# Adamtaranto/frisk

Hardware: AMD Instinct MI355X
Metric: windows/sec (k=1..8, w=5kb, s=1kb) (higher is better)
Workload: dtype u8/u4 counts + f64 scores

## Files before the change

### frisk_amd/csrc/frisk_abi.hip

```cpp
#include <hip/hip_runtime.h>
#include <zlib.h>
#include <dlfcn.h>

#include <algorithm>
#include <cmath>
#include <cstdio>
#include <cstdlib>
#include <cstring>
#include <new>
#include <string>
#include <atomic>
#include <chrono>
#include <thread>
#include <vector>

#include "frisk_hip.h"
#include "frisk_device.h"
#include "profile_kernels.h"
#include "scan_launch.h"
#include "scan_schedule.h"
#include "ring_rows.h"
#include "synth_kernel.h"
#include "table_text.h"
#include "fasta_index.h"
// ... 10 lines not shown
    hipError_t reserve(size_t n) {
        if (n <= cap) return hipSuccess;
        if (p) { hipError_t e = hipFree(p); p = nullptr; cap = 0; if (e != hipSuccess) return e; }
        size_t want = n + n / 8 + 64;
        hipError_t e = hipMalloc(reinterpret_cast<void**>(&p), want * sizeof(T));
        if (e != hipSuccess) { p = nullptr; return e; }
        cap = want;
        return hipSuccess;
    }
    void release() { if (p) (void)hipFree(p); p = nullptr; cap = 0; }
};

}

struct frisk_ctx {
    int device = 0;
    int kmin = 1, kmax = 8;
    int64_t nprof = 0;
    int num_cu = 256;
    hipStream_t stream = nullptr;
    hipEvent_t ev0 = nullptr, ev1 = nullptr;
    double ms[3] = {-1.0, -1.0, -1.0};
    std::string err;

    struct Batch {
        int32_t n_seq = 0;
        std::vector<int64_t> seq_off, seq_len;
        std::vector<std::string> seq_name;
        int64_t padded_len = 0;
        bool have_seq = false;
        DevBuf<uint8_t> d_ascii;
        DevBuf<uint32_t> d_codes, d_inv, d_low;
        struct Tile {
            int32_t scaf;
            int64_t size;
            int64_t base0;
            int64_t j0, ncand;
            int32_t kind;
            int64_t own0, own1;
        };
        int width_hint = 0, hint_w = 0, hint_inc = 0, hint_side = 0;
        bool tiled = false;
        std::vector<Tile> tiles;
        int32_t tile_w = 0, tile_inc = 0;
        uint32_t tile_flags = 0;
        int64_t cand_begin = 0, cand_end = 0;
        std::vector<std::string> g_name;
        std::vector<int64_t> g_len;
        std::vector<int64_t> piece_end;
        std::vector<hipEvent_t> piece_ev;
        bool streaming = false;
        DevBuf<int64_t> d_runs;
        std::vector<uint32_t, frisk_fasta::NoInitAlloc<uint32_t>> h_codes;
        frisk_pack2::Runs h_runs;
        bool have_host2 = false;
        int64_t* h_pads = nullptr;
        size_t h_pads_cap = 0;
        void release() {
            d_ascii.release(); d_codes.release(); d_inv.release(); d_low.release(); d_runs.release();
            if (h_pads) (void)hipHostFree(h_pads);
            h_pads = nullptr; h_pads_cap = 0;
            for (hipEvent_t e : piece_ev) (void)hipEventDestroy(e);
            piece_ev.clear();
        }
    };
    Batch bat[2];
    int cur = 0;
    Batch& b() { return bat[cur]; }
    const Batch& b() const { return bat[cur]; }
    hipStream_t copy_stream = nullptr;
    static constexpr int PIN_N = 8;
    static constexpr size_t PIN_BYTES = size_t(16) << 20;
    void* pin_buf[PIN_N] = {nullptr, nullptr, nullptr, nullptr, nullptr, nullptr, nullptr, nullptr};
    hipEvent_t pin_ev[PIN_N] = {nullptr, nullptr, nullptr, nullptr, nullptr, nullptr, nullptr, nullptr};
    bool pin_busy[PIN_N] = {false, false, false, false, false, false, false, false};
    hipStream_t tail_stream = nullptr;
    hipEvent_t ev_fork = nullptr, ev_tail_kernels = nullptr, ev_tail_done = nullptr;
    hipEvent_t staged_ev = nullptr;
    hipEvent_t slot_free_ev = nullptr;
    bool slot_ev_set = false;
    bool staged = false;

    DevBuf<int64_t> d_raw, d_cnt, d_sym;
    DevBuf<double> d_ig, d_logtab, d_logtab64, d_logtab32, d_rctab;
    DevBuf<int64_t> d_ovf_list, d_ovf_list2;
    uint64_t ig_gen = 1, ring_gen = 0;
    DevBuf<double> d_ig_ring;
    DevBuf<unsigned int> d_verdict;
    DevBuf<unsigned int> d_ovf_count;
    int64_t scan_stat[5] = {0, 0, 0, 0, 0};
    DevBuf<uint32_t> d_big;
    DevBuf<int64_t> d_meta;
    int64_t* h_meta = nullptr;
    bool profile_final = false;
    bool ms_pending[3] = {false, false, false};
    hipEvent_t evp0 = nullptr, evp1 = nullptr;

    DevBuf<ScafDesc> d_desc;
    std::vector<ScafDesc> h_desc;
    int32_t plan_w = -1, plan_inc = -1;
    uint32_t plan_flags = 0;
    int64_t plan_ncand = 0;
    int64_t plan_maxwin = 0;
    DevBuf<int32_t> o_seq;
    DevBuf<int64_t> o_start, o_stop, o_meta;
    DevBuf<uint32_t> o_status, o_counts;
    DevBuf<double> o_kld, o_gc, o_pi, o_si, o_cri, o_sw, o_sg, o_ivom;
    DevBuf<double> o_block;
    void* h_block = nullptr;
    size_t h_block_cap = 0;
    double* want_ivom = nullptr;
};

namespace {

int fail(frisk_ctx* c, int code, const std::string& msg) {
    if (c) c->err = msg;
    return code;
}

#define HIPC(ctx, call)                                                                         \
    do {                                                                                        \
        hipError_t e_ = (call);                                                                 \
        if (e_ != hipSuccess)                                                                   \
            return fail((ctx), FRISK_E_HIP, std::string(#call) + ": " + hipGetErrorString(e_)); \
    } while (0)

int64_t profile_len(int kmin, int kmax) { return table_offset(kmin, kmax + 1); }

int grid_for(int64_t items, int per_block, int max_blocks) {
    int64_t b = (items + per_block - 1) / per_block;
    if (b < 1) b = 1;
    if (b > max_blocks) b = max_blocks;
    return int(b);
}

int settle_stream(frisk_ctx* c);

int layout_batch(frisk_ctx* c, frisk_ctx::Batch& B, const int64_t* lens, int32_t n_seq) {
    if (n_seq < 0) return fail(c, FRISK_E_ARG, "n_seq < 0");
    for (int32_t s = 0; s < n_seq; ++s)
        if (lens[s] < 0) return fail(c, FRISK_E_ARG, "negative scaffold length");
    if (&B == &c->b()) {
        const int rc = settle_stream(c);
        if (rc) return rc;
    }
    B.seq_off.assign(size_t(n_seq), 0);
    B.seq_len.assign(lens, lens + n_seq);
    B.seq_name.assign(size_t(n_seq), std::string());
    int64_t pos = 0;
    for (int32_t s = 0; s < n_seq; ++s) {
        B.seq_off[size_t(s)] = pos;
        pos += lens[s] + 1;
    }
    B.padded_len = (pos + 31) / 32 * 32;
    if (B.padded_len == 0) B.padded_len = 32;
    B.n_seq = n_seq;
    B.have_seq = false;
    B.width_hint = 0;
    B.tiled = false;
    B.tiles.clear(); B.g_name.clear(); B.g_len.clear();
    B.streaming = false;
    if (B.have_host2) {
        B.have_host2 = false;
        decltype(B.h_codes)().swap(B.h_codes);
        B.h_runs = frisk_pack2::Runs();
// ... 177 lines not shown

}

extern "C" {

const char* frisk_version(void) { return "frisk_hip 0.1 (gfx950)"; }

int frisk_supported(int kmin, int kmax, int64_t max_window) {
    return (kmin >= 1 && kmin <= kmax && kmax <= FRISK_MAX_K && max_window >= 1 && max_window <= 0x7FFFFFFF) ? 1 : 0;
}

int frisk_create(int device, int kmin, int kmax, frisk_ctx** out) {
    if (!out) return FRISK_E_ARG;
    *out = nullptr;
    frisk_ctx* c = new (std::nothrow) frisk_ctx();
    if (!c) return FRISK_E_HIP;
    *out = c;
    if (kmin < 1 || kmin > kmax || kmax > FRISK_MAX_K)
        return fail(c, FRISK_E_ARG, "word sizes must satisfy 1 <= kmin <= kmax <= 12");
    c->device = device;
    c->kmin = kmin;
    c->kmax = kmax;
    c->nprof = profile_len(kmin, kmax);
    int ndev = 0;
    HIPC(c, hipGetDeviceCount(&ndev));
    if (device < 0 || device >= ndev) return fail(c, FRISK_E_HIP, "no such HIP device");
    HIPC(c, hipSetDevice(device));
    hipDeviceProp_t prop;
    HIPC(c, hipGetDeviceProperties(&prop, device));
    if (std::string(prop.gcnArchName).rfind("gfx950", 0) != 0)
        return fail(c, FRISK_E_HIP, std::string("libfrisk_hip is built for gfx950 only; device is ") + prop.gcnArchName);
    c->num_cu = prop.multiProcessorCount;
    HIPC(c, hipStreamCreateWithFlags(&c->stream, hipStreamNonBlocking));
    HIPC(c, hipStreamCreateWithFlags(&c->copy_stream, hipStreamNonBlocking));
    HIPC(c, hipEventCreateWithFlags(&c->staged_ev, hipEventDisableTiming));
    HIPC(c, hipEventCreateWithFlags(&c->slot_free_ev, hipEventDisableTiming));
    HIPC(c, hipStreamCreateWithFlags(&c->tail_stream, hipStreamNonBlocking));
    HIPC(c, hipEventCreateWithFlags(&c->ev_fork, hipEventDisableTiming));
    HIPC(c, hipEventCreateWithFlags(&c->ev_tail_kernels, hipEventDisableTiming));
    HIPC(c, hipEventCreateWithFlags(&c->ev_tail_done, hipEventDisableTiming));
    HIPC(c, hipEventCreate(&c->ev0));
    HIPC(c, hipEventCreate(&c->ev1));
    HIPC(c, c->d_raw.reserve(size_t(c->nprof) + 4));
    HIPC(c, c->d_cnt.reserve(size_t(c->nprof) + 4));
    HIPC(c, c->d_sym.reserve(size_t(c->nprof)));
    HIPC(c, c->d_ig.reserve(size_t(1) << (2 * kmax)));
    HIPC(c, c->d_meta.reserve(4));
    HIPC(c, hipHostMalloc(reinterpret_cast<void**>(&c->h_meta), 4 * sizeof(int64_t), hipHostMallocDefault));
    HIPC(c, hipEventCreate(&c->evp0));
    HIPC(c, hipEventCreate(&c->evp1));
    HIPC(c, hipMemsetAsync(c->d_raw.p, 0, (size_t(c->nprof) + 4) * sizeof(int64_t), c->stream));
    {
        double tab[2 * FRISK_LOGTAB_N];
        for (int nbin : {FRISK_LOGTAB_N, 64, 32}) {
            for (int i = 0; i < nbin; ++i) {
                const double ci = 0.5 + (double(i) + 0.5) / (2.0 * nbin);
                const double u = 1.0 / ci;
                tab[2 * i] = u;
                tab[2 * i + 1] = double(-logl((long double)u));
            }
            DevBuf<double>& dst = nbin == 64 ? c->d_logtab64 : (nbin == 32 ? c->d_logtab32 : c->d_logtab);
            HIPC(c, dst.reserve(2 * size_t(nbin)));
            HIPC(c, hipMemcpyAsync(dst.p, tab, 2 * size_t(nbin) * sizeof(double), hipMemcpyHostToDevice, c->stream));
            HIPC(c, hipStreamSynchronize(c->stream));
        }
        double rc[256];
        rc[0] = 0.0;
        for (int i = 1; i < 256; ++i) rc[i] = 1.0 / double(i);
        HIPC(c, c->d_rctab.reserve(256));
        HIPC(c, hipMemcpyAsync(c->d_rctab.p, rc, sizeof(rc), hipMemcpyHostToDevice, c->stream));
        HIPC(c, c->d_ovf_count.reserve(64));
        HIPC(c, c->d_verdict.reserve(8));
        HIPC(c, hipStreamSynchronize(c->stream));
    }
    HIPC(c, hipStreamSynchronize(c->stream));
    return FRISK_OK;
}

void frisk_destroy(frisk_ctx* c) {
    if (!c) return;
    (void)hipSetDevice(c->device);
    if (c->stream) (void)hipStreamSynchronize(c->stream);
    c->bat[0].release(); c->bat[1].release();
    c->d_raw.release(); c->d_cnt.release(); c->d_sym.release(); c->d_ig.release(); c->d_logtab.release(); c->d_logtab64.release(); c->d_logtab32.release(); c->d_rctab.release(); c->d_ig_ring.release(); c->d_ovf_list.release(); c->d_ovf_list2.release(); c->d_ovf_count.release(); c->d_verdict.release(); c->d_big.release(); c->d_desc.release();
    c->o_seq.release(); c->o_start.release(); c->o_stop.release(); c->o_meta.release();
    c->o_status.release(); c->o_counts.release();
    c->o_ivom.release(); c->o_kld.release(); c->o_gc.release(); c->o_sw.release(); c->o_sg.release(); c->o_pi.release(); c->o_si.release(); c->o_cri.release();
    if (c->copy_stream) { (void)hipStreamSynchronize(c->copy_stream); (void)hipStreamDestroy(c->copy_stream); }
    if (c->staged_ev) (void)hipEventDestroy(c->staged_ev);
    if (c->slot_free_ev) (void)hipEventDestroy(c->slot_free_ev);
    for (int i = 0; i < frisk_ctx::PIN_N; ++i) {
        if (c->pin_ev[i]) { (void)hipEventSynchronize(c->pin_ev[i]); (void)hipEventDestroy(c->pin_ev[i]); }
        if (c->pin_buf[i]) (void)hipHostFree(c->pin_buf[i]);
    }
    if (c->tail_stream) { (void)hipStreamSynchronize(c->tail_stream); (void)hipStreamDestroy(c->tail_stream); }
    if (c->ev_fork) (void)hipEventDestroy(c->ev_fork);
    if (c->ev_tail_kernels) (void)hipEventDestroy(c->ev_tail_kernels);
    if (c->ev_tail_done) (void)hipEventDestroy(c->ev_tail_done);
    if (c->h_meta) (void)hipHostFree(c->h_meta);
    if (c->h_block) (void)hipHostFree(c->h_block);
    c->o_block.release();
    if (c->evp0) (void)hipEventDestroy(c->evp0);
    if (c->evp1) (void)hipEventDestroy(c->evp1);
    c->d_meta.release();
    if (c->ev0) (void)hipEventDestroy(c->ev0);
    if (c->ev1) (void)hipEventDestroy(c->ev1);
    if (c->stream) (void)hipStreamDestroy(c->stream);
    delete c;
}

const char* frisk_last_error(const frisk_ctx* c) { return c ? c->err.c_str() : "null context"; }
int64_t frisk_profile_len(const frisk_ctx* c) { return c ? c->nprof : 0; }
int64_t frisk_profile_raw_len(const frisk_ctx* c) { return c ? c->nprof + 4 : 0; }
int64_t frisk_seq_padded_len(const frisk_ctx* c) { return (c && c->b().have_seq) ? c->b().padded_len : 0; }
void* frisk_host_alloc(frisk_ctx* c, int64_t bytes) {
    if (!c || bytes <= 0) return nullptr;
    void* p = nullptr;
    if (hipSetDevice(c->device) != hipSuccess) return nullptr;
    if (hipHostMalloc(&p, size_t(bytes), hipHostMallocDefault) != hipSuccess) { c->err = "hipHostMalloc failed"; return nullptr; }
    return p;
}
void frisk_host_free(frisk_ctx* c, void* ptr) {
    if (c && ptr) { (void)hipSetDevice(c->device); (void)hipHostFree(ptr); }
}
double frisk_last_kernel_ms(const frisk_ctx* cc, int which) {
    frisk_ctx* c = const_cast<frisk_ctx*>(cc);
    if (!c || which < 0 || which >= 3) return -1.0;
    if (which == 1 && c->ms_pending[1]) {
        float ms = 0;
        if (hipEventSynchronize(c->evp1) == hipSuccess && hipEventElapsedTime(&ms, c->evp0, c->evp1) == hipSuccess) c->ms[1] = ms;
        c->ms_pending[1] = false;
    }
    return c->ms[which];
}

int frisk_seq_load(frisk_ctx* c, const uint8_t* const* seqs, const int64_t* lens, int32_t n_seq) {
    if (!c) return FRISK_E_ARG;
    if (n_seq > 0 && (!seqs || !lens)) return fail(c, FRISK_E_ARG, "null sequence table");
    HIPC(c, hipSetDevice(c->device));
    int rc = layout_batch(c, lens, n_seq);
    if (rc) return rc;
    if (n_seq <= 64) {
        rc = enqueue_ascii_upload(c, c->b(), seqs, lens, n_seq, c->stream);
        if (rc) return rc;
    } else {
        HIPC(c, c->b().d_ascii.reserve(size_t(c->b().padded_len)));
        std::vector<uint8_t> stage(size_t(c->b().padded_len), uint8_t(FRISK_PAD_BYTE));
        for (int32_t s = 0; s < n_seq; ++s)
            if (lens[s] > 0) std::memcpy(stage.data() + c->b().seq_off[size_t(s)], seqs[s], size_t(lens[s]));
        rc = h2d(c, c->b().d_ascii.p, stage.data(), stage.size(), c->stream);
        if (rc) return rc;
        HIPC(c, hipStreamSynchronize(c->stream));
    }
    rc = alloc_packed(c);
    if (rc) return rc;
    return run_pack(c);
}

int frisk_fasta_pack_2bit(const char* path, int32_t* n_seq, int64_t** lens, uint32_t** codes, int64_t* n_code_words, int64_t** inv_runs,
                          int64_t* n_inv, int64_t** low_runs, int64_t* n_low) {
    if (!path || !n_seq || !lens || !codes || !n_code_words || !inv_runs || !n_inv || !low_runs || !n_low) return FRISK_E_ARG;
    frisk_fasta::Records rec;
    frisk_fasta::CodeVec packed;
    frisk_pack2::Runs R;
    std::string err;
    const unsigned hw = std::thread::hardware_concurrency();
    if (!frisk_fasta::parse_pack(path, rec, packed, R, err, int(std::min(32u, hw ? hw : 1u)))) return FRISK_E_ARG;
// ... 473 lines not shown
int frisk_seq_export_packed(frisk_ctx* c, uint32_t* codes, uint32_t* inv, uint32_t* low) {
    if (!c || !codes || !inv || !low) return FRISK_E_ARG;
    if (!c->b().have_seq) return fail(c, FRISK_E_STATE, "no resident sequence batch");
    HIPC(c, hipSetDevice(c->device));
    if (int rs = settle_stream(c)) return rs;
    const size_t w32 = size_t(c->b().padded_len / 32);
    HIPC(c, hipMemcpyAsync(codes, c->b().d_codes.p, 2 * w32 * 4, hipMemcpyDeviceToHost, c->stream));
    HIPC(c, hipMemcpyAsync(inv, c->b().d_inv.p, w32 * 4, hipMemcpyDeviceToHost, c->stream));
    HIPC(c, hipMemcpyAsync(low, c->b().d_low.p, w32 * 4, hipMemcpyDeviceToHost, c->stream));
    HIPC(c, hipStreamSynchronize(c->stream));
    return FRISK_OK;
}

int frisk_seq_set_names(frisk_ctx* c, const char* const* names, int32_t n_seq) {
    if (!c || (n_seq > 0 && !names)) return FRISK_E_ARG;
    if (!c->b().have_seq || n_seq != c->b().n_seq) return fail(c, FRISK_E_ARG, "frisk_seq_set_names: one name per resident scaffold");
    for (int32_t s = 0; s < n_seq; ++s) c->b().seq_name[size_t(s)] = names[s] ? names[s] : "";
    return FRISK_OK;
}

int frisk_seq_synth(frisk_ctx* c, const int64_t* lens, int32_t n_seq, uint64_t seed, double island_frac,
                    double n_frac, double lower_frac, double repeats_per_kb) {
    return frisk_seq_synth2(c, lens, n_seq, seed, island_frac, n_frac, lower_frac, repeats_per_kb, 0.0, 0.0);
}

int frisk_seq_synth2(frisk_ctx* c, const int64_t* lens, int32_t n_seq, uint64_t seed, double island_frac,
                     double n_frac, double lower_frac, double repeats_per_kb, double period_mix, double sat_frac) {
    if (!c) return FRISK_E_ARG;
    if (n_seq > 0 && !lens) return fail(c, FRISK_E_ARG, "null length table");
    HIPC(c, hipSetDevice(c->device));
    int rc = layout_batch(c, lens, n_seq);
    if (rc) return rc;
    HIPC(c, c->b().d_ascii.reserve(size_t(c->b().padded_len)));
    HIPC(c, hipMemsetAsync(c->b().d_ascii.p, FRISK_PAD_BYTE, size_t(c->b().padded_len), c->stream));
    SynthTables tabs;
    synth_make_tables(seed, tabs);
    const uint32_t thr_island = synth_frac_to_u32(island_frac), thr_nbig = synth_frac_to_u32(n_frac * 0.8),
                   thr_nsmall = synth_frac_to_u32(n_frac * 0.2), thr_low = synth_frac_to_u32(lower_frac),
                   thr_rep = synth_frac_to_u32(repeats_per_kb * (SYNTH_REP / 1000.0)), thr_mix = synth_frac_to_u32(period_mix),
                   thr_sat = synth_frac_to_u32(sat_frac * (2.0 * SYNTH_SAT_GROUP / (SYNTH_SAT_GROUP + 1.0))),
                   thr_div = synth_frac_to_u32(SYNTH_SAT_DIV);
    for (int32_t s = 0; s < n_seq; ++s) {
        if (lens[s] <= 0) continue;
        const int64_t nblk = (lens[s] + SYNTH_BLOCK - 1) / SYNTH_BLOCK;
        synth_kernel<<<grid_for(nblk, 64, 1 << 20), 64, 0, c->stream>>>(c->b().d_ascii.p + c->b().seq_off[size_t(s)], lens[s],
                                                                       seed, uint32_t(s), tabs, thr_island, thr_nbig,
                                                                       thr_nsmall, thr_low, thr_rep, thr_mix, thr_sat, thr_div);
        HIPC(c, hipGetLastError());
    }
    rc = alloc_packed(c);
    if (rc) return rc;
    return run_pack(c);
}

int frisk_seq_read(frisk_ctx* c, int32_t s, int64_t offset, int64_t n, uint8_t* out) {
    if (!c || !out) return FRISK_E_ARG;
    if (!c->b().have_seq) return fail(c, FRISK_E_STATE, "no resident sequence batch");
    if (c->b().tiled) return fail(c, FRISK_E_STATE, "frisk_seq_read: the resident batch holds tiles, not whole scaffolds");
    if (s < 0 || s >= c->b().n_seq) return fail(c, FRISK_E_ARG, "sequence index out of range");
    if (offset < 0 || n < 0 || offset + n > c->b().seq_len[size_t(s)]) return fail(c, FRISK_E_ARG, "range outside the scaffold");
    if (n == 0) return FRISK_OK;
    HIPC(c, hipSetDevice(c->device));
    if (int rs = settle_stream(c)) return rs;
    DevBuf<uint8_t> tmp;
    HIPC(c, tmp.reserve(size_t(n)));
    unpack_kernel<<<grid_for(n, 256, c->num_cu * 8), 256, 0, c->stream>>>(c->b().d_codes.p, c->b().d_inv.p, c->b().d_low.p,
                                                                           c->b().seq_off[size_t(s)] + offset, n, tmp.p);
    hipError_t e = hipGetLastError();
    if (e == hipSuccess) e = hipMemcpyAsync(out, tmp.p, size_t(n), hipMemcpyDeviceToHost, c->stream);
    if (e == hipSuccess) e = hipStreamSynchronize(c->stream);
    tmp.release();
    HIPC(c, e);
    return FRISK_OK;
}

int frisk_profile_reset(frisk_ctx* c) {
    if (!c) return FRISK_E_ARG;
    HIPC(c, hipSetDevice(c->device));
    HIPC(c, hipMemsetAsync(c->d_raw.p, 0, (size_t(c->nprof) + 4) * sizeof(int64_t), c->stream));
    c->profile_final = false;
    return FRISK_OK;
}

static int profile_add_range(frisk_ctx* c, int mask_host, bool one_pass, int64_t p0, int64_t p1, bool first = true, bool last = true);

int frisk_profile_add(frisk_ctx* c, int mask_host, int64_t p0, int64_t p1) {
    if (!c) return FRISK_E_ARG;
    const bool one_pass = (mask_host & FRISK_PROFILE_ONE_PASS) != 0;
    mask_host &= 1;
    if (!c->b().have_seq) return fail(c, FRISK_E_STATE, "frisk_profile_add: no resident sequence batch");
    if (c->b().tiled) {
        if (!(p0 < 0 && p1 < 0)) return fail(c, FRISK_E_ARG, "frisk_profile_add: a tiled batch is profiled as a whole (-1, -1)");
        c->profile_final = false;
        const frisk_ctx::Batch& B = c->b();
        for (size_t t = 0; t < B.tiles.size(); ++t) {
            const frisk_ctx::Batch::Tile& T = B.tiles[t];
            if (T.own1 <= T.own0) continue;
            int rc = profile_add_range(c, mask_host, one_pass, B.seq_off[t] + (T.own0 - T.base0), B.seq_off[t] + (T.own1 - T.base0));
            if (rc) return rc;
        }
        return FRISK_OK;
    }
    frisk_ctx::Batch& SB = c->b();
    if (SB.streaming && p0 < 0 && p1 < 0 && !SB.piece_end.empty()) {
        HIPC(c, hipSetDevice(c->device));
        const size_t np = SB.piece_end.size();
        int64_t done = 0;
        for (size_t i = 0; i < np; ++i) {
            HIPC(c, hipStreamWaitEvent(c->stream, SB.piece_ev[i], 0));
            const int64_t upto = i + 1 == np ? SB.padded_len : (SB.piece_end[i] - 1) * 32;
            if (upto > done || i + 1 == np || i == 0) {
                int rc = profile_add_range(c, mask_host, one_pass, done, std::max(done, upto), i == 0, i + 1 == np);
                if (rc) return rc;
                done = std::max(done, upto);
            }
        }
        SB.streaming = false;
        return FRISK_OK;
    }
    if (int rs = settle_stream(c)) return rs;
    return profile_add_range(c, mask_host, one_pass, p0, p1);
}

static int profile_add_range(frisk_ctx* c, int mask_host, bool one_pass, int64_t p0, int64_t p1, bool first, bool last) {
    if (p0 < 0 && p1 < 0) { p0 = 0; p1 = c->b().padded_len; }
    if (p0 < 0 || p1 > c->b().padded_len || p0 > p1) return fail(c, FRISK_E_ARG, "position range outside the batch");
    HIPC(c, hipSetDevice(c->device));
    c->profile_final = false;
    if (c->kmax > 8) {
        const int64_t nw = p1 > p0 ? ((p1 + 31) >> 5) - (p0 >> 5) : 0;
        if (first) HIPC(c, hipEventRecord(c->evp0, c->stream));
        if (nw > 0)
            profile_add_big_kernel<<<grid_for(nw, 256, c->num_cu * 8), 256, 0, c->stream>>>(
                c->b().d_codes.p, c->b().d_inv.p, c->b().d_low.p, p0, p1, c->kmin, c->kmax, mask_host ? 1 : 0, int(c->nprof),
                reinterpret_cast<unsigned long long*>(c->d_raw.p));
        HIPC(c, hipGetLastError());
        if (last) { HIPC(c, hipEventRecord(c->evp1, c->stream)); c->ms_pending[1] = true; }
        return FRISK_OK;
    }
    if (c->kmax == 8 && (one_pass || p1 - p0 >= (int64_t(1) << 30))) {
        const int64_t span16 = p1 - p0;
        const int64_t nwords16 = span16 > 0 ? ((p1 + 31) >> 5) - (p0 >> 5) : 0;
        int64_t nch = std::min<int64_t>(std::max<int64_t>(1, span16 / 65536), int64_t(c->num_cu));
        const int64_t chunk_len16 = (nwords16 + nch - 1) / std::max<int64_t>(nch, 1);
        nch = chunk_len16 > 0 ? (nwords16 + chunk_len16 - 1) / chunk_len16 : 0;
        if (first) HIPC(c, hipEventRecord(c->evp0, c->stream));
        if (span16 > 0) {
            HIPC(c, hipFuncSetAttribute(reinterpret_cast<const void*>(profile_add16_kernel), hipFuncAttributeMaxDynamicSharedMemorySize, 131072));
            profile_add16_kernel<<<int(nch), FRISK_PROF_NT, 131072, c->stream>>>(c->b().d_codes.p, c->b().d_inv.p, c->b().d_low.p, p0, p1, c->kmin,
                                                                                 mask_host ? 1 : 0, int(c->nprof), chunk_len16,
                                                                                 reinterpret_cast<unsigned long long*>(c->d_raw.p));
        }
        HIPC(c, hipGetLastError());
        if (last) { HIPC(c, hipEventRecord(c->evp1, c->stream)); c->ms_pending[1] = true; }
        return FRISK_OK;
    }
    const int halves = (c->kmax == 8) ? 2 : 1;
    const size_t lds = (size_t(1) << (2 * c->kmax)) / size_t(halves) * 4;
    const int64_t span = p1 - p0;
    const int64_t nwords = span > 0 ? ((p1 + 31) >> 5) - (p0 >> 5) : 0;
    constexpr int64_t wg_per_cu = 1;
    int64_t nchunks = std::min<int64_t>(std::max<int64_t>(1, span / 65536), int64_t(c->num_cu) * wg_per_cu / halves);
    const int64_t chunk_len = (nwords + nchunks - 1) / std::max<int64_t>(nchunks, 1);
    nchunks = chunk_len > 0 ? (nwords + chunk_len - 1) / chunk_len : 0;
    if (first) HIPC(c, hipEventRecord(c->evp0, c->stream));
    if (span > 0) {
        auto raw = reinterpret_cast<unsigned long long*>(c->d_raw.p);
        HIPC(c, hipFuncSetAttribute(reinterpret_cast<const void*>(profile_add_kernel),
                                    hipFuncAttributeMaxDynamicSharedMemorySize, int(std::max<size_t>(lds, 16))));
        profile_add_kernel<<<int(nchunks) * halves, FRISK_PROF_NT, std::max<size_t>(lds, 16), c->stream>>>(
            c->b().d_codes.p, c->b().d_inv.p, c->b().d_low.p, p0, p1, c->kmin, c->kmax, mask_host ? 1 : 0, int(c->nprof), halves,
            chunk_len, raw);
    }
    HIPC(c, hipGetLastError());
    if (last) {
        HIPC(c, hipEventRecord(c->evp1, c->stream));
        c->ms_pending[1] = true;
    }
    return FRISK_OK;
}

int frisk_profile_export_device(frisk_ctx* c, void* dst) {
    if (!c || !dst) return FRISK_E_ARG;
    HIPC(c, hipSetDevice(c->device));
    HIPC(c, hipMemcpyAsync(dst, c->d_raw.p, (size_t(c->nprof) + 4) * 8, hipMemcpyDeviceToDevice, c->stream));
    HIPC(c, hipStreamSynchronize(c->stream));
    return FRISK_OK;
}
int frisk_profile_import_device(frisk_ctx* c, const void* src) {
    if (!c || !src) return FRISK_E_ARG;
    HIPC(c, hipSetDevice(c->device));
    HIPC(c, hipMemcpyAsync(c->d_raw.p, src, (size_t(c->nprof) + 4) * 8, hipMemcpyDeviceToDevice, c->stream));
    HIPC(c, hipStreamSynchronize(c->stream));
    c->profile_final = false;
    return FRISK_OK;
}
int frisk_profile_device_view(frisk_ctx* c, void** raw, void** stream) {
    if (!c || !raw || !stream) return FRISK_E_ARG;
    *raw = c->d_raw.p;
    *stream = reinterpret_cast<void*>(c->stream);
    c->profile_final = false;
    return FRISK_OK;
}
int frisk_profile_allreduce(frisk_ctx* c, void* rccl_comm) {
    if (!c) return FRISK_E_ARG;
    if (!rccl_comm) return FRISK_OK;
    typedef int (*allreduce_fn)(const void*, void*, size_t, int, int, void*, hipStream_t);
    typedef const char* (*errstr_fn)(int);
    static allreduce_fn all_reduce = nullptr;
    static errstr_fn err_string = nullptr;
    if (!all_reduce) {
        void* h = dlopen("librccl.so.1", RTLD_NOW | RTLD_NOLOAD);
        if (!h) h = dlopen("librccl.so.1", RTLD_NOW | RTLD_GLOBAL);
        if (!h) h = dlopen("librccl.so", RTLD_NOW | RTLD_GLOBAL);
        if (!h) return fail(c, FRISK_E_HIP, std::string("frisk_profile_allreduce: librccl not found: ") + dlerror());
        all_reduce = reinterpret_cast<allreduce_fn>(dlsym(h, "ncclAllReduce"));
        err_string = reinterpret_cast<errstr_fn>(dlsym(h, "ncclGetErrorString"));
        if (!all_reduce) return fail(c, FRISK_E_HIP, "frisk_profile_allreduce: ncclAllReduce not found in librccl");
    }
    HIPC(c, hipSetDevice(c->device));
    const int rc = all_reduce(c->d_raw.p, c->d_raw.p, size_t(c->nprof) + 4,  4,  0, rccl_comm, c->stream);
    if (rc != 0) return fail(c, FRISK_E_HIP, std::string("ncclAllReduce: ") + (err_string ? err_string(rc) : "error"));
    c->profile_final = false;
    return FRISK_OK;
}

int frisk_profile_export_host(frisk_ctx* c, int64_t* dst) {
    if (!c || !dst) return FRISK_E_ARG;
    HIPC(c, hipSetDevice(c->device));
    HIPC(c, hipMemcpyAsync(dst, c->d_raw.p, (size_t(c->nprof) + 4) * 8, hipMemcpyDeviceToHost, c->stream));
    HIPC(c, hipStreamSynchronize(c->stream));
    return FRISK_OK;
}
int frisk_profile_import_host(frisk_ctx* c, const int64_t* src) {
    if (!c || !src) return FRISK_E_ARG;
    HIPC(c, hipSetDevice(c->device));
    HIPC(c, hipMemcpyAsync(c->d_raw.p, src, (size_t(c->nprof) + 4) * 8, hipMemcpyHostToDevice, c->stream));
    HIPC(c, hipStreamSynchronize(c->stream));
    c->profile_final = false;
    return FRISK_OK;
}
// ... 476 lines not shown
```

### frisk_amd/csrc/profile_kernels.h

```cpp
#pragma once
#include "frisk_device.h"

__device__ inline void classify_byte(uint32_t c, uint32_t& code, uint32_t& inv, uint32_t& low) {
    const uint32_t u = c & 0xDFu;
    const uint32_t isA = (u == 'A'), isT = (u == 'T'), isG = (u == 'G'), isC = (u == 'C');
    const uint32_t valid = isA | isT | isG | isC;
    code = isT * 1u + isG * 2u + isC * 3u;
    const uint32_t is_pad = (c == FRISK_PAD_BYTE);
    inv = (valid ^ 1u);
    low = (valid & ((c >> 5) & 1u)) | is_pad;
}

__global__ __launch_bounds__(256) void pack_kernel(const uint8_t* __restrict__ ascii, int64_t nwords32,
                                                    uint32_t* __restrict__ codes, uint32_t* __restrict__ inv,
                                                    uint32_t* __restrict__ low) {
    const int64_t stride = int64_t(gridDim.x) * blockDim.x;
    for (int64_t t = int64_t(blockIdx.x) * blockDim.x + threadIdx.x; t < nwords32; t += stride) {
        const uint4* src = reinterpret_cast<const uint4*>(ascii + t * 32);
        const uint4 q0 = src[0], q1 = src[1];
        const uint32_t w[8] = {q0.x, q0.y, q0.z, q0.w, q1.x, q1.y, q1.z, q1.w};
        uint32_t c0 = 0, c1 = 0, mi = 0, ml = 0;
#pragma unroll
        for (int b = 0; b < 32; ++b) {
            const uint32_t ch = (w[b >> 2] >> (8 * (b & 3))) & 0xFFu;
            uint32_t code, i1, l1;
            classify_byte(ch, code, i1, l1);
            if (b < 16) c0 |= code << (30 - 2 * b); else c1 |= code << (30 - 2 * (b - 16));
            mi |= i1 << (31 - b);
            ml |= l1 << (31 - b);
        }
        codes[2 * t] = c0;
        codes[2 * t + 1] = c1;
        inv[t] = mi;
        low[t] = ml;
    }
}

__global__ __launch_bounds__(256) void unpack_kernel(const uint32_t* __restrict__ codes,
                                                      const uint32_t* __restrict__ inv,
                                                      const uint32_t* __restrict__ low, int64_t p0, int64_t n,
                                                      uint8_t* __restrict__ out) {
    const int64_t stride = int64_t(gridDim.x) * blockDim.x;
    for (int64_t t = int64_t(blockIdx.x) * blockDim.x + threadIdx.x; t < n; t += stride) {
        const int64_t g = p0 + t;
        const uint32_t i1 = fetch_mask1(inv, g), l1 = fetch_mask1(low, g), c = fetch_code2(codes, g);
        uint8_t ch;
        if (i1 && l1) ch = 0;
        else if (i1) ch = 'N';
        else ch = uint8_t("ATGC"[c] | (l1 ? 0x20 : 0));
        out[t] = ch;
    }
}

__global__ __launch_bounds__(256) void expand_runs_kernel(const int64_t* __restrict__ runs, int64_t n_runs,
                                                           uint32_t* __restrict__ bits) {
    const int lane = int(threadIdx.x & 63u);
    const int64_t wave = (int64_t(blockIdx.x) * blockDim.x + threadIdx.x) >> 6;
    const int64_t nwaves = (int64_t(gridDim.x) * blockDim.x) >> 6;
    for (int64_t r = wave; r < n_runs; r += nwaves) {
        const int64_t b = runs[2 * r], e = runs[2 * r + 1];
        if (e <= b) continue;
        const int64_t w0 = b >> 5, w1 = (e - 1) >> 5;
        for (int64_t w = w0 + lane; w <= w1; w += 64) {
            const int64_t lo = w << 5;
            const int from = b > lo ? int(b - lo) : 0, to = e < lo + 32 ? int(e - lo) : 32;
            const uint32_t m = uint32_t((0xFFFFFFFFull >> from) & ~(0xFFFFFFFFull >> to));
            if (m == 0xFFFFFFFFu) bits[w] = m;
            else atomicOr(bits + w, m);
        }
    }
}

#define FRISK_PROF_NT 1024

__global__ __launch_bounds__(FRISK_PROF_NT) void profile_add_kernel(const uint32_t* __restrict__ codes,
                                                                     const uint32_t* __restrict__ inv,
                                                                     const uint32_t* __restrict__ low, int64_t p0, int64_t p1,
                                                                     int kmin, int kmax, int mask_host, int nprof,
                                                                     int halves, int64_t chunk_words,
                                                                     unsigned long long* __restrict__ raw) {
    extern __shared__ __attribute__((aligned(16))) uint32_t hist[];
    const int half = int(blockIdx.x) % halves;
    const int64_t chunk = int64_t(blockIdx.x) / halves;
    const uint32_t nbins = (1u << (2 * kmax)) / uint32_t(halves);
    for (uint32_t b = threadIdx.x; b < nbins / 4; b += blockDim.x) reinterpret_cast<uint4*>(hist)[b] = make_uint4(0, 0, 0, 0);
    if (nbins < 4) for (uint32_t b = threadIdx.x; b < nbins; b += blockDim.x) hist[b] = 0;
    __syncthreads();
    unsigned long long tot = 0, kpos = 0, nn = 0;
    const int64_t w_first = p0 >> 5, w_end = (p1 + 31) >> 5;
    const int64_t wb = w_first + chunk * chunk_words;
    int64_t we = wb + chunk_words;
    if (we > w_end) we = w_end;
    const int64_t offK = table_offset(kmin, kmax);
    const int shK = 16 - 2 * kmax;
    const uint32_t halfbit = (halves == 2) ? nbins : 0u;
    auto topbits = [](int64_t k) -> uint32_t {
        k = k < 0 ? 0 : (k > 32 ? 32 : k);
        return uint32_t(0xFFFFFFFF00000000ull >> k);
    };
    for (int64_t wq = wb + threadIdx.x; wq < we; wq += blockDim.x) {
        const int64_t base = wq << 5;
        const uint32_t i0 = inv[wq], i1 = inv[wq + 1], l0 = low[wq], l1 = low[wq + 1];
        const uint32_t c0 = codes[2 * wq], c1 = codes[2 * wq + 1], c2 = codes[2 * wq + 2];
        const uint32_t inr = topbits(p1 - base) & ~topbits(p0 - base);
        const uint32_t e0 = i0 | (mask_host ? l0 : 0u), e1 = i1 | (mask_host ? l1 : 0u);
        const uint64_t V = ~((uint64_t(e0) << 32) | e1);
        uint64_t F = V;
        for (int s = 1; s < kmax; ++s) F &= V << s;
        const uint32_t fullm = uint32_t(F >> 32) & inr;
        const uint64_t lo64 = (uint64_t(c0) << 32) | c1, hi64 = (uint64_t(c1) << 32) | c2;
#pragma unroll
        for (int j = 0; j < 32; ++j) {
            if (fullm & (0x80000000u >> j)) {
                const uint32_t c16 = uint32_t((j < 16 ? lo64 : hi64) >> (48 - 2 * (j & 15))) & 0xFFFFu;
                const uint32_t code = c16 >> shK;
                if ((code & halfbit) == (half ? halfbit : 0u)) atomicAdd(&hist[code & (nbins - 1)], 1u);
            }
        }
        if (half == 0) {
            uint32_t shortm = uint32_t(V >> 32) & ~uint32_t(F >> 32) & inr;
            while (shortm) {
                const int j = __clz(int(shortm));
                shortm &= ~(0x80000000u >> j);
                const int run = __clzll((long long)(~(V << j)));
                if (run >= kmin) {
                    const uint32_t c16 = uint32_t((j < 16 ? lo64 : hi64) >> (48 - 2 * (j & 15))) & 0xFFFFu;
                    atomicAdd(&raw[table_offset(kmin, run) + (c16 >> (16 - 2 * run))], 1ull);
                }
            }
            const uint64_t NP = ~((uint64_t(i0 & l0) << 32) | (i1 & l1));
            uint64_t G = NP;
            for (int s = 1; s < kmax; ++s) G &= NP << s;
            const uint32_t real = uint32_t(NP >> 32) & inr;
            tot += __popc(real);
            nn += __popc(real & (i0 | l0));
            kpos += __popc(uint32_t(G >> 32) & inr);
        }
    }
    if (half == 0) {
        for (int o = 32; o > 0; o >>= 1) {
            tot += __shfl_down(tot, o);
            kpos += __shfl_down(kpos, o);
            nn += __shfl_down(nn, o);
        }
        if ((threadIdx.x & 63) == 0) {
            if (tot) atomicAdd(&raw[nprof + 0], tot);
            if (kpos) atomicAdd(&raw[nprof + 1], kpos);
            if (nn) atomicAdd(&raw[nprof + 2], nn);
        }
    }
    __syncthreads();
    for (uint32_t b = threadIdx.x; b < nbins; b += blockDim.x) {
        const uint32_t v = hist[b];
        if (v) atomicAdd(&raw[offK + uint32_t(half) * nbins + b], (unsigned long long)v);
    }
}

__global__ __launch_bounds__(FRISK_PROF_NT) void profile_add16_kernel(const uint32_t* __restrict__ codes,
                                                                       const uint32_t* __restrict__ inv,
                                                                       const uint32_t* __restrict__ low, int64_t p0, int64_t p1,
                                                                       int kmin, int mask_host, int nprof, int64_t chunk_words,
                                                                       unsigned long long* __restrict__ raw) {
    constexpr int K = 8;
    constexpr uint32_t NW = (1u << (2 * K)) / 2;
    extern __shared__ __attribute__((aligned(16))) uint32_t hist[];
    __shared__ unsigned long long red[2];
    const int64_t chunk = int64_t(blockIdx.x);
    auto clear = [&]() {
        for (uint32_t b = threadIdx.x; b < NW / 4; b += blockDim.x) reinterpret_cast<uint4*>(hist)[b] = make_uint4(0, 0, 0, 0);
    };
    clear();
    if (threadIdx.x < 2) red[threadIdx.x] = 0ull;
    __syncthreads();
    const int64_t w_first = p0 >> 5, w_end = (p1 + 31) >> 5;
    const int64_t wb = w_first + chunk * chunk_words;
    int64_t we = wb + chunk_words;
    if (we > w_end) we = w_end;
    const int64_t offK = table_offset(kmin, K);
    auto topbits = [](int64_t k) -> uint32_t {
        k = k < 0 ? 0 : (k > 32 ? 32 : k);
        return uint32_t(0xFFFFFFFF00000000ull >> k);
    };
    auto walk = [&](auto mode_c) {
        constexpr int MODE = decltype(mode_c)::value;
        unsigned long long tot = 0, kpos = 0, nn = 0, mine = 0;
        for (int64_t wq = wb + threadIdx.x; wq < we; wq += blockDim.x) {
            const int64_t base = wq << 5;
            const uint32_t i0 = inv[wq], i1 = inv[wq + 1], l0 = low[wq], l1 = low[wq + 1];
            const uint32_t c0 = codes[2 * wq], c1 = codes[2 * wq + 1], c2 = codes[2 * wq + 2];
            const uint32_t inr = topbits(p1 - base) & ~topbits(p0 - base);
            const uint32_t e0 = i0 | (mask_host ? l0 : 0u), e1 = i1 | (mask_host ? l1 : 0u);
            const uint64_t V = ~((uint64_t(e0) << 32) | e1);
            uint64_t F = V;
            F &= F << 1; F &= F << 2; F &= F << 4;
            const uint32_t fullm = uint32_t(F >> 32) & inr;
            const uint64_t lo64 = (uint64_t(c0) << 32) | c1, hi64 = (uint64_t(c1) << 32) | c2;
#pragma unroll
            for (int j = 0; j < 32; ++j) {
                if (fullm & (0x80000000u >> j)) {
                    const uint32_t code = uint32_t((j < 16 ? lo64 : hi64) >> (48 - 2 * (j & 15))) & 0xFFFFu;
                    if (MODE == 0) atomicAdd(&hist[code >> 1], 1u << ((code & 1u) * 16u));
                    else if ((code >> 15) == uint32_t(MODE - 1)) atomicAdd(&hist[code & (NW - 1u)], 1u);
                }
            }
            if (MODE == 0) {
                mine += uint32_t(__popc(fullm));
                uint32_t shortm = uint32_t(V >> 32) & ~uint32_t(F >> 32) & inr;
                while (shortm) {
                    const int j = __clz(int(shortm));
                    shortm &= ~(0x80000000u >> j);
                    const int run = __clzll((long long)(~(V << j)));
                    if (run >= kmin) {
                        const uint32_t c16 = uint32_t((j < 16 ? lo64 : hi64) >> (48 - 2 * (j & 15))) & 0xFFFFu;
                        atomicAdd(&raw[table_offset(kmin, run) + (c16 >> (16 - 2 * run))], 1ull);
                    }
                }
                const uint64_t NP = ~((uint64_t(i0 & l0) << 32) | (i1 & l1));
                uint64_t G = NP;
                G &= G << 1; G &= G << 2; G &= G << 4;
                const uint32_t real = uint32_t(NP >> 32) & inr;
                tot += __popc(real);
                nn += __popc(real & (i0 | l0));
                kpos += __popc(uint32_t(G >> 32) & inr);
            }
        }
        if (MODE == 0) {
            for (int o = 32; o > 0; o >>= 1) {
                tot += __shfl_down(tot, o); kpos += __shfl_down(kpos, o); nn += __shfl_down(nn, o); mine += __shfl_down(mine, o);
            }
            if ((threadIdx.x & 63) == 0) {
                if (tot) atomicAdd(&raw[nprof + 0], tot);
                if (kpos) atomicAdd(&raw[nprof + 1], kpos);
                if (nn) atomicAdd(&raw[nprof + 2], nn);
                if (mine) atomicAdd(&red[0], mine);
            }
        }
    };
    walk(std::integral_constant<int, 0>{});
    __syncthreads();
    {
        unsigned long long sum = 0;
        for (uint32_t b = threadIdx.x; b < NW; b += blockDim.x) { const uint32_t v = hist[b]; sum += (v & 0xFFFFu) + (v >> 16); }
        for (int o = 32; o > 0; o >>= 1) sum += __shfl_down(sum, o);
        if ((threadIdx.x & 63) == 0 && sum) atomicAdd(&red[1], sum);
    }
    __syncthreads();
    if (red[0] == red[1]) {
        for (uint32_t b = threadIdx.x; b < NW; b += blockDim.x) {
            const uint32_t v = hist[b];
            if (v & 0xFFFFu) atomicAdd(&raw[offK + 2u * b], (unsigned long long)(v & 0xFFFFu));
            if (v >> 16) atomicAdd(&raw[offK + 2u * b + 1u], (unsigned long long)(v >> 16));
        }
        return;
    }
    for (int half = 0; half < 2; ++half) {
        __syncthreads();
        clear();
        __syncthreads();
        if (half == 0) walk(std::integral_constant<int, 1>{}); else walk(std::integral_constant<int, 2>{});
        __syncthreads();
        for (uint32_t b = threadIdx.x; b < NW; b += blockDim.x) {
            const uint32_t v = hist[b];
            if (v) atomicAdd(&raw[offK + uint32_t(half) * NW + b], (unsigned long long)v);
        }
    }
}

__global__ __launch_bounds__(256) void profile_add_big_kernel(const uint32_t* __restrict__ codes, const uint32_t* __restrict__ inv,
                                                               const uint32_t* __restrict__ low, int64_t p0, int64_t p1, int kmin,
                                                               int kmax, int mask_host, int nprof,
                                                               unsigned long long* __restrict__ raw) {
    unsigned long long tot = 0, kpos = 0, nn = 0;
    const int64_t w_first = p0 >> 5, w_end = (p1 + 31) >> 5;
    auto topbits = [](int64_t k) -> uint32_t {
        k = k < 0 ? 0 : (k > 32 ? 32 : k);
        return uint32_t(0xFFFFFFFF00000000ull >> k);
    };
    for (int64_t wq = w_first + int64_t(blockIdx.x) * blockDim.x + threadIdx.x; wq < w_end; wq += int64_t(gridDim.x) * blockDim.x) {
        const int64_t base = wq << 5;
        const uint32_t i0 = inv[wq], i1 = inv[wq + 1], l0 = low[wq], l1 = low[wq + 1];
        const uint32_t c0 = codes[2 * wq], c1 = codes[2 * wq + 1], c2 = codes[2 * wq + 2];
        const uint32_t inr = topbits(p1 - base) & ~topbits(p0 - base);
        const uint32_t e0 = i0 | (mask_host ? l0 : 0u), e1 = i1 | (mask_host ? l1 : 0u);
        const uint64_t V = ~((uint64_t(e0) << 32) | e1);
        const uint64_t lo64 = (uint64_t(c0) << 32) | c1, hi64 = (uint64_t(c1) << 32) | c2;
        uint32_t todo = uint32_t(V >> 32) & inr;
        while (todo) {
            const int j = __clz(int(todo));
            todo &= ~(0x80000000u >> j);
            int run = __clzll((long long)(~(V << j)));
            run = run < kmax ? run : kmax;
            if (run >= kmin) {
                const uint32_t c24 = uint32_t((j < 16 ? lo64 : hi64) >> (40 - 2 * (j & 15))) & 0xFFFFFFu;
                atomicAdd(&raw[table_offset(kmin, run) + (c24 >> (24 - 2 * run))], 1ull);
            }
        }
        const uint64_t NP = ~((uint64_t(i0 & l0) << 32) | (i1 & l1));
        uint64_t G = NP;
        for (int s = 1; s < kmax; ++s) G &= NP << s;
        const uint32_t real = uint32_t(NP >> 32) & inr;
        tot += __popc(real);
        nn += __popc(real & (i0 | l0));
        kpos += __popc(uint32_t(G >> 32) & inr);
    }
    for (int o = 32; o > 0; o >>= 1) {
        tot += __shfl_down(tot, o);
        kpos += __shfl_down(kpos, o);
        nn += __shfl_down(nn, o);
    }
    if ((threadIdx.x & 63) == 0) {
        if (tot) atomicAdd(&raw[nprof + 0], tot);
        if (kpos) atomicAdd(&raw[nprof + 1], kpos);
        if (nn) atomicAdd(&raw[nprof + 2], nn);
    }
}

__global__ __launch_bounds__(256) void marginalize_kernel(int64_t* __restrict__ cnt, int kmin, int x) {
    const int64_t q = int64_t(blockIdx.x) * blockDim.x + threadIdx.x;
    if (q >= (int64_t(1) << (2 * x))) return;
    const int64_t* up = cnt + table_offset(kmin, x + 1) + 4 * q;
    cnt[table_offset(kmin, x) + q] += up[0] + up[1] + up[2] + up[3];
}

__global__ __launch_bounds__(1024) void marginalize_low_kernel(int64_t* __restrict__ cnt, int kmin, int x_hi) {
    for (int x = x_hi; x >= kmin; --x) {
        const int64_t n = int64_t(1) << (2 * x);
        int64_t* dst = cnt + table_offset(kmin, x);
        const int64_t* up = cnt + table_offset(kmin, x + 1);
        for (int64_t q = threadIdx.x; q < n; q += blockDim.x) dst[q] += up[4 * q] + up[4 * q + 1] + up[4 * q + 2] + up[4 * q + 3];
        __threadfence_block();
        __syncthreads();
    }
}

__global__ __launch_bounds__(256) void symmetrize_kernel(const int64_t* __restrict__ fwd, int64_t* __restrict__ sym,
                                                          int kmin, int kmax) {
    const int64_t t = int64_t(blockIdx.x) * blockDim.x + threadIdx.x;
    for (int x = kmin; x <= kmax; ++x) {
        const int64_t off = table_offset(kmin, x), n = int64_t(1) << (2 * x);
        if (t >= off && t < off + n) {
            const uint32_t c = uint32_t(t - off);
            sym[t] = fwd[t] + fwd[off + revcomp_code(c, x)];
        }
    }
}

#pragma clang fp contract(off)
// ... 40 lines not shown
```

Measured before the change: 66.32 million.

## Route all k=8 profiles through one-pass LDS kernel with dump-and-reduce flush

For kmax=8 the one-pass 16-bit-packed LDS histogram kernel now always runs, where before it was used only on request or for very large spans, so the two-half fallback is dropped from the default path. Each workgroup now writes its packed histogram as a per-slot dump in global memory plus a validity flag, replacing per-bin global 64-bit atomics, and a new reduce kernel sums slots per bin before a smaller atomic flush into raw. A wave-uniform fast path skips per-bit mask checks when every position in the word is a full k-mer. The cost is an extra kernel launch and a global scratch buffer sized per CU.

```diff
diff --git a/frisk_amd/csrc/frisk_abi.hip b/frisk_amd/csrc/frisk_abi.hip
--- a/frisk_amd/csrc/frisk_abi.hip
+++ b/frisk_amd/csrc/frisk_abi.hip
@@ -116,6 +116,7 @@
     bool staged = false;
 
     DevBuf<int64_t> d_raw, d_cnt, d_sym;
+    DevBuf<uint32_t> d_prof_dump;
     DevBuf<double> d_ig, d_logtab, d_logtab64, d_logtab32, d_rctab;
     DevBuf<int64_t> d_ovf_list, d_ovf_list2;
     uint64_t ig_gen = 1, ring_gen = 0;
@@ -459,7 +460,7 @@
     (void)hipSetDevice(c->device);
     if (c->stream) (void)hipStreamSynchronize(c->stream);
     c->bat[0].release(); c->bat[1].release();
-    c->d_raw.release(); c->d_cnt.release(); c->d_sym.release(); c->d_ig.release(); c->d_logtab.release(); c->d_logtab64.release(); c->d_logtab32.release(); c->d_rctab.release(); c->d_ig_ring.release(); c->d_ovf_list.release(); c->d_ovf_list2.release(); c->d_ovf_count.release(); c->d_verdict.release(); c->d_big.release(); c->d_desc.release();
+    c->d_raw.release(); c->d_prof_dump.release(); c->d_cnt.release(); c->d_sym.release(); c->d_ig.release(); c->d_logtab.release(); c->d_logtab64.release(); c->d_logtab32.release(); c->d_rctab.release(); c->d_ig_ring.release(); c->d_ovf_list.release(); c->d_ovf_list2.release(); c->d_ovf_count.release(); c->d_verdict.release(); c->d_big.release(); c->d_desc.release();
     c->o_seq.release(); c->o_start.release(); c->o_stop.release(); c->o_meta.release();
     c->o_status.release(); c->o_counts.release();
     c->o_ivom.release(); c->o_kld.release(); c->o_gc.release(); c->o_sw.release(); c->o_sg.release(); c->o_pi.release(); c->o_si.release(); c->o_cri.release();
@@ -1099,11 +1100,10 @@
     return FRISK_OK;
 }
 
-static int profile_add_range(frisk_ctx* c, int mask_host, bool one_pass, int64_t p0, int64_t p1, bool first = true, bool last = true);
+static int profile_add_range(frisk_ctx* c, int mask_host, int64_t p0, int64_t p1, bool first = true, bool last = true);
 
 int frisk_profile_add(frisk_ctx* c, int mask_host, int64_t p0, int64_t p1) {
     if (!c) return FRISK_E_ARG;
-    const bool one_pass = (mask_host & FRISK_PROFILE_ONE_PASS) != 0;
     mask_host &= 1;
     if (!c->b().have_seq) return fail(c, FRISK_E_STATE, "frisk_profile_add: no resident sequence batch");
     if (c->b().tiled) {
@@ -1113,7 +1113,7 @@
         for (size_t t = 0; t < B.tiles.size(); ++t) {
             const frisk_ctx::Batch::Tile& T = B.tiles[t];
             if (T.own1 <= T.own0) continue;
-            int rc = profile_add_range(c, mask_host, one_pass, B.seq_off[t] + (T.own0 - T.base0), B.seq_off[t] + (T.own1 - T.base0));
+            int rc = profile_add_range(c, mask_host, B.seq_off[t] + (T.own0 - T.base0), B.seq_off[t] + (T.own1 - T.base0));
             if (rc) return rc;
         }
         return FRISK_OK;
@@ -1127,7 +1127,7 @@
             HIPC(c, hipStreamWaitEvent(c->stream, SB.piece_ev[i], 0));
             const int64_t upto = i + 1 == np ? SB.padded_len : (SB.piece_end[i] - 1) * 32;
             if (upto > done || i + 1 == np || i == 0) {
-                int rc = profile_add_range(c, mask_host, one_pass, done, std::max(done, upto), i == 0, i + 1 == np);
+                int rc = profile_add_range(c, mask_host, done, std::max(done, upto), i == 0, i + 1 == np);
                 if (rc) return rc;
                 done = std::max(done, upto);
             }
@@ -1136,10 +1136,10 @@
         return FRISK_OK;
     }
     if (int rs = settle_stream(c)) return rs;
-    return profile_add_range(c, mask_host, one_pass, p0, p1);
-}
-
-static int profile_add_range(frisk_ctx* c, int mask_host, bool one_pass, int64_t p0, int64_t p1, bool first, bool last) {
+    return profile_add_range(c, mask_host, p0, p1);
+}
+
+static int profile_add_range(frisk_ctx* c, int mask_host, int64_t p0, int64_t p1, bool first, bool last) {
     if (p0 < 0 && p1 < 0) { p0 = 0; p1 = c->b().padded_len; }
     if (p0 < 0 || p1 > c->b().padded_len || p0 > p1) return fail(c, FRISK_E_ARG, "position range outside the batch");
     HIPC(c, hipSetDevice(c->device));
@@ -1155,7 +1155,7 @@
         if (last) { HIPC(c, hipEventRecord(c->evp1, c->stream)); c->ms_pending[1] = true; }
         return FRISK_OK;
     }
-    if (c->kmax == 8 && (one_pass || p1 - p0 >= (int64_t(1) << 30))) {
+    if (c->kmax == 8) {
         const int64_t span16 = p1 - p0;
         const int64_t nwords16 = span16 > 0 ? ((p1 + 31) >> 5) - (p0 >> 5) : 0;
         int64_t nch = std::min<int64_t>(std::max<int64_t>(1, span16 / 65536), int64_t(c->num_cu));
@@ -1163,17 +1163,25 @@
         nch = chunk_len16 > 0 ? (nwords16 + chunk_len16 - 1) / chunk_len16 : 0;
         if (first) HIPC(c, hipEventRecord(c->evp0, c->stream));
         if (span16 > 0) {
-            HIPC(c, hipFuncSetAttribute(reinterpret_cast<const void*>(profile_add16_kernel), hipFuncAttributeMaxDynamicSharedMemorySize, 131072));
-            profile_add16_kernel<<<int(nch), FRISK_PROF_NT, 131072, c->stream>>>(c->b().d_codes.p, c->b().d_inv.p, c->b().d_low.p, p0, p1, c->kmin,
-                                                                                 mask_host ? 1 : 0, int(c->nprof), chunk_len16,
-                                                                                 reinterpret_cast<unsigned long long*>(c->d_raw.p));
+            const size_t max_slots = size_t(std::max(c->num_cu, 1));
+            HIPC(c, c->d_prof_dump.reserve(max_slots * FRISK_PROF16_WORDS + max_slots));
+            uint32_t* dump = c->d_prof_dump.p;
+            uint32_t* valid = dump + max_slots * FRISK_PROF16_WORDS;
+            auto raw = reinterpret_cast<unsigned long long*>(c->d_raw.p);
+            HIPC(c, hipFuncSetAttribute(reinterpret_cast<const void*>(profile_add16_kernel), hipFuncAttributeMaxDynamicSharedMemorySize, FRISK_PROF16_LDS));
+            profile_add16_kernel<<<int(nch), FRISK_PROF_NT, FRISK_PROF16_LDS, c->stream>>>(c->b().d_codes.p, c->b().d_inv.p, c->b().d_low.p, p0, p1, c->kmin,
+                                                                                 mask_host ? 1 : 0, int(c->nprof), chunk_len16, raw, dump, valid);
+            HIPC(c, hipGetLastError());
+            const int split = int(std::min<int64_t>(FRISK_PROF_RED_SPLIT, nch));
+            profile_reduce16_kernel<<<dim3(FRISK_PROF16_QUADS / FRISK_PROF_RED_NT, split), FRISK_PROF_RED_NT, 0, c->stream>>>(
+                dump, valid, int(nch), table_offset(c->kmin, 8), raw);
         }
         HIPC(c, hipGetLastError());
         if (last) { HIPC(c, hipEventRecord(c->evp1, c->stream)); c->ms_pending[1] = true; }
         return FRISK_OK;
     }
-    const int halves = (c->kmax == 8) ? 2 : 1;
-    const size_t lds = (size_t(1) << (2 * c->kmax)) / size_t(halves) * 4;
+    constexpr int halves = 1;
+    const size_t lds = (size_t(1) << (2 * c->kmax)) * 4;
     const int64_t span = p1 - p0;
     const int64_t nwords = span > 0 ? ((p1 + 31) >> 5) - (p0 >> 5) : 0;
     constexpr int64_t wg_per_cu = 1;
diff --git a/frisk_amd/csrc/profile_flush.h b/frisk_amd/csrc/profile_flush.h
--- /dev/null
+++ b/frisk_amd/csrc/profile_flush.h
@@ -0,0 +1,44 @@
+#pragma once
+
+#include <cstddef>
+#include <cstdint>
+
+#if defined(__HIPCC__)
+#define FRISK_FLUSH_FN __host__ __device__ inline
+#else
+#define FRISK_FLUSH_FN inline
+#endif
+
+#define FRISK_PROF16_WORDS 32768u
+#define FRISK_PROF16_QUADS (FRISK_PROF16_WORDS / 4u)
+
+struct alignas(16) ProfQuad { uint32_t w[4]; };
+
+FRISK_FLUSH_FN uint32_t prof16_word(uint32_t code) { return code >> 1; }
+FRISK_FLUSH_FN uint32_t prof16_field(uint32_t code) { return code & 1u; }
+FRISK_FLUSH_FN uint32_t prof16_inc(uint32_t code) { return 1u << (prof16_field(code) * 16u); }
+FRISK_FLUSH_FN uint32_t prof16_code(uint32_t word, uint32_t field) { return 2u * word + field; }
+
+FRISK_FLUSH_FN size_t prof_slot_off(uint32_t slot) { return size_t(slot) * FRISK_PROF16_WORDS; }
+FRISK_FLUSH_FN uint32_t prof_group_begin(uint32_t nslots, uint32_t split, uint32_t g) {
+    const uint32_t per = (nslots + split - 1u) / split;
+    const uint64_t b = uint64_t(g) * per;
+    return b < nslots ? uint32_t(b) : nslots;
+}
+FRISK_FLUSH_FN uint32_t prof_quad_bin(uint32_t quad, uint32_t j, uint32_t field) { return prof16_code(4u * quad + j, field); }
+
+FRISK_FLUSH_FN void prof_reduce_quad(const uint32_t* __restrict__ dump, const uint32_t* __restrict__ valid, uint32_t nslots, uint32_t split,
+                                     uint32_t g, uint32_t quad, unsigned long long sums[8]) {
+    for (int i = 0; i < 8; ++i) sums[i] = 0ull;
+    const uint32_t s0 = prof_group_begin(nslots, split, g), s1 = prof_group_begin(nslots, split, g + 1u);
+#pragma unroll 8
+    for (uint32_t s = s0; s < s1; ++s) {
+        const ProfQuad q = *reinterpret_cast<const ProfQuad*>(dump + prof_slot_off(s) + 4u * quad);
+        const uint32_t m = valid[s] ? 0xFFFFFFFFu : 0u;
+        for (int j = 0; j < 4; ++j) {
+            const uint32_t w = q.w[j] & m;
+            sums[2 * j] += w & 0xFFFFu;
+            sums[2 * j + 1] += w >> 16;
+        }
+    }
+}
diff --git a/frisk_amd/csrc/profile_kernels.h b/frisk_amd/csrc/profile_kernels.h
--- a/frisk_amd/csrc/profile_kernels.h
+++ b/frisk_amd/csrc/profile_kernels.h
@@ -1,5 +1,6 @@
 #pragma once
 #include "frisk_device.h"
+#include "profile_flush.h"
 
 __device__ inline void classify_byte(uint32_t c, uint32_t& code, uint32_t& inv, uint32_t& low) {
     const uint32_t u = c & 0xDFu;
@@ -156,13 +157,15 @@
     }
 }
 
+#define FRISK_PROF16_LDS (FRISK_PROF16_WORDS * 4u)
 __global__ __launch_bounds__(FRISK_PROF_NT) void profile_add16_kernel(const uint32_t* __restrict__ codes,
                                                                        const uint32_t* __restrict__ inv,
                                                                        const uint32_t* __restrict__ low, int64_t p0, int64_t p1,
                                                                        int kmin, int mask_host, int nprof, int64_t chunk_words,
-                                                                       unsigned long long* __restrict__ raw) {
+                                                                       unsigned long long* __restrict__ raw,
+                                                                       uint32_t* __restrict__ dump, uint32_t* __restrict__ valid) {
     constexpr int K = 8;
-    constexpr uint32_t NW = (1u << (2 * K)) / 2;
+    constexpr uint32_t NW = FRISK_PROF16_WORDS;
     extern __shared__ __attribute__((aligned(16))) uint32_t hist[];
     __shared__ unsigned long long red[2];
     const int64_t chunk = int64_t(blockIdx.x);
@@ -195,12 +198,20 @@
             F &= F << 1; F &= F << 2; F &= F << 4;
             const uint32_t fullm = uint32_t(F >> 32) & inr;
             const uint64_t lo64 = (uint64_t(c0) << 32) | c1, hi64 = (uint64_t(c1) << 32) | c2;
-#pragma unroll
-            for (int j = 0; j < 32; ++j) {
-                if (fullm & (0x80000000u >> j)) {
+            if (MODE == 0 && __all(fullm == 0xFFFFFFFFu)) {
+#pragma unroll
+                for (int j = 0; j < 32; ++j) {
                     const uint32_t code = uint32_t((j < 16 ? lo64 : hi64) >> (48 - 2 * (j & 15))) & 0xFFFFu;
-                    if (MODE == 0) atomicAdd(&hist[code >> 1], 1u << ((code & 1u) * 16u));
-                    else if ((code >> 15) == uint32_t(MODE - 1)) atomicAdd(&hist[code & (NW - 1u)], 1u);
+                    atomicAdd(&hist[prof16_word(code)], prof16_inc(code));
+                }
+            } else {
+#pragma unroll
+                for (int j = 0; j < 32; ++j) {
+                    if (fullm & (0x80000000u >> j)) {
+                        const uint32_t code = uint32_t((j < 16 ? lo64 : hi64) >> (48 - 2 * (j & 15))) & 0xFFFFu;
+                        if (MODE == 0) atomicAdd(&hist[prof16_word(code)], prof16_inc(code));
+                        else if ((code >> 15) == uint32_t(MODE - 1)) atomicAdd(&hist[code & (NW - 1u)], 1u);
+                    }
                 }
             }
             if (MODE == 0) {
@@ -246,13 +257,12 @@
     }
     __syncthreads();
     if (red[0] == red[1]) {
-        for (uint32_t b = threadIdx.x; b < NW; b += blockDim.x) {
-            const uint32_t v = hist[b];
-            if (v & 0xFFFFu) atomicAdd(&raw[offK + 2u * b], (unsigned long long)(v & 0xFFFFu));
-            if (v >> 16) atomicAdd(&raw[offK + 2u * b + 1u], (unsigned long long)(v >> 16));
-        }
+        ProfQuad* slot = reinterpret_cast<ProfQuad*>(dump + prof_slot_off(blockIdx.x));
+        for (uint32_t b = threadIdx.x; b < FRISK_PROF16_QUADS; b += blockDim.x) slot[b] = reinterpret_cast<const ProfQuad*>(hist)[b];
+        if (threadIdx.x == 0) valid[blockIdx.x] = 1u;
         return;
     }
+    if (threadIdx.x == 0) valid[blockIdx.x] = 0u;
     for (int half = 0; half < 2; ++half) {
         __syncthreads();
         clear();
@@ -263,6 +273,27 @@
             const uint32_t v = hist[b];
             if (v) atomicAdd(&raw[offK + uint32_t(half) * NW + b], (unsigned long long)v);
         }
+    }
+}
+
+#define FRISK_PROF_RED_NT 256
+#define FRISK_PROF_RED_SPLIT 8
+static_assert(FRISK_PROF16_QUADS % FRISK_PROF_RED_NT == 0, "profile_reduce16_kernel: whole workgroups of quads");
+__global__ __launch_bounds__(FRISK_PROF_RED_NT) void profile_reduce16_kernel(const uint32_t* __restrict__ dump,
+                                                                              const uint32_t* __restrict__ valid, int nslots,
+                                                                              int64_t offK, unsigned long long* __restrict__ raw) {
+    __shared__ unsigned long long tr[FRISK_PROF_RED_NT * 8];
+    const uint32_t quad0 = blockIdx.x * FRISK_PROF_RED_NT;
+    unsigned long long sums[8];
+    prof_reduce_quad(dump, valid, uint32_t(nslots), gridDim.y, blockIdx.y, quad0 + threadIdx.x, sums);
+#pragma unroll
+    for (uint32_t i = 0; i < 8; ++i) tr[prof_quad_bin(threadIdx.x, i >> 1, i & 1u)] = sums[i];
+    __syncthreads();
+    unsigned long long* dst = raw + offK + prof_quad_bin(quad0, 0, 0);
+#pragma unroll
+    for (uint32_t i = 0; i < 8; ++i) {
+        const uint32_t k = i * FRISK_PROF_RED_NT + threadIdx.x;
+        atomicAdd(dst + k, tr[k]);
     }
 }
 
```

Result: no change. 66.98 million (median of 6 runs) (+1.0%).
